# wanmeihuali/taichi_3d_gaussian_splatting

Hardware: NVIDIA H100
Metric: rendered Mpix/sec fwd+bwd @1080p, 1e6 Gaussians (higher is better)
Workload: dtype f32

## Files before the change

### taichi_3d_gaussian_splatting_b200/csrc/blend_bwd.cu

```cuda
#include "blend_bwd.cuh"

namespace gsb {

__device__ __forceinline__ void warp_transpose_reduce11(float (&v)[11], int lane) {
    {
        const bool hi = lane & 16;
#pragma unroll
        for (int i = 0; i < 5; ++i) {
            const float send = hi ? v[i] : v[i + 6];
            const float keep = hi ? v[i + 6] : v[i];
            v[i] = keep + __shfl_xor_sync(0xffffffffu, send, 16);
        }
        v[5] += __shfl_xor_sync(0xffffffffu, v[5], 16);
    }
    {
        const bool hi = lane & 8;
#pragma unroll
        for (int i = 0; i < 3; ++i) {
            const float send = hi ? v[i] : v[i + 3];
            const float keep = hi ? v[i + 3] : v[i];
            v[i] = keep + __shfl_xor_sync(0xffffffffu, send, 8);
        }
    }
    {
// ... 138 lines not shown
                            v[3] = vs0 * q1;
                            v[4] = vs1 * q1;
                            v[5] = aT * g0;
                            v[6] = aT * g1;
                            v[7] = aT * g2;
                            v[8] = a_grad * gp * (1.0f - opa) * opa;
                            v[9] = STATS ? sqrtf(vs0 * vs0 + vs1 * vs1) : 0.0f;
                        } else {
                            const float P = fast_alpha(d0, d1, (-0.5f * GSB_L2E) * r0.z, -GSB_L2E * r0.w,
                                                       (-0.5f * GSB_L2E) * r1.x, r1.y);
                            contributes = (idx < last) && (P >= 1.0f / 255.0f);
                            const float alpha = fminf(P, 0.99f);
                            const float inv = rcp_approx(1.0f - alpha);
                            const float Tn = T * inv;
                            const float aT = contributes ? alpha * Tn : 0.0f;
                            const float cg = fmaf(r2.z, g2, fmaf(r2.y, g1, r2.x * g0));
                            const float a_grad = contributes ? fmaf(cg, Tn, -(w0 * inv)) : 0.0f;
                            T = contributes ? Tn : T;
                            w0 = fmaf(cg, aT, w0);
                            const float G = a_grad * P;
                            const float vs0 = G * q0, vs1 = G * q1;
                            if (STATS) {
                                mag0 += fabsf(vs0);
                                mag1 += fabsf(vs1);
                            }
                            v[0] = vs0;
                            v[1] = vs1;
                            v[2] = vs0 * q0;
                            v[3] = vs0 * q1;
                            v[4] = vs1 * q1;
                            v[5] = aT * g0;
                            v[6] = aT * g1;
                            v[7] = aT * g2;
                            v[8] = G * r1.z;
                            v[9] = STATS ? sqrt_approx(vs0 * vs0 + vs1 * vs1) : 0.0f;
                        }
                        v[10] = (STATS && contributes) ? 1.0f : 0.0f;
                    }
                    if (lane == 0) GSB_EMU_COUNT(EC_BF_VISITS, 1);
                    GSB_EMU_COUNT(EC_BF_PAIRS, contributes ? 1 : 0);
                    if (__any_sync(0xffffffffu, contributes)) {
                        if (lane == 0) GSB_EMU_COUNT(EC_BF_VISITS_ANY, 1);
                        warp_transpose_reduce11(v, lane);
                        if (red_writer && (STATS || red_slot < 9))
                            atomicAdd(p.accum + (size_t)s_off[buf][j] * GSB_ACCUM_FLOATS + red_slot, v[0]);
                    }
                }
            }
        }
    }
    if (STATS) {
        p.mag_image[2 * pix] = mag0;
        p.mag_image[2 * pix + 1] = mag1;
    }
}

#ifndef GSB_HOST_EMU
static BlendBwdParams make_blend_bwd_params(const GsbBackwardArgs &a, const Workspace &ws);

int launch_blend_backward_work(const GsbBackwardArgs &a, const Workspace &ws, unsigned long long *counters_dev,
                               cudaStream_t stream) {
    BlendBwdParams p = make_blend_bwd_params(a, ws);
    p.work_counters = counters_dev;
    const int tiles = p.tiles_x * (a.camera_height / GSB_TILE_HEIGHT);
    if (tiles <= 0) return GSB_OK;
    return launch_blend_backward_count(p, tiles, stream);
}

static BlendBwdParams make_blend_bwd_params(const GsbBackwardArgs &a, const Workspace &ws) {
    BlendBwdParams p;
    p.H = a.camera_height;
    p.W = a.camera_width;
    p.tiles_x = a.camera_width / GSB_TILE_WIDTH;
    p.tile_start = ws.tile_start;
    p.tile_end = ws.tile_end;
    p.sorted_vals = ws.vals_b;
    p.records = ws.records;
    p.grad_image = a.grad_rasterized_image;
    p.acc_alpha = a.pixel_accumulated_alpha;
    p.last_effective = a.pixel_offset_of_last_effective_point;
    p.accum = a.accum;
    p.mag_image = a.magnitude_grad_viewspace_on_image;
    p.work_counters = nullptr;
    p.grad_depth = nullptr;
    p.depth = nullptr;
    p.grad_alpha = nullptr;
    return p;
}

int launch_blend_backward(const GsbBackwardArgs &a, const Workspace &ws, cudaStream_t stream, const float *grad_depth,
                          const float *depth, const float *grad_alpha, const GsbExtraFeatureArgs *ext) {
    BlendBwdParams p;
    p.H = a.camera_height;
    p.W = a.camera_width;
    p.tiles_x = a.camera_width / GSB_TILE_WIDTH;
    p.tile_start = ws.tile_start;
    p.tile_end = ws.tile_end;
    p.sorted_vals = ws.vals_b;
    p.records = ws.records;
    p.grad_image = a.grad_rasterized_image;
    p.acc_alpha = a.pixel_accumulated_alpha;
    p.last_effective = a.pixel_offset_of_last_effective_point;
    p.accum = a.accum;
    p.mag_image = a.magnitude_grad_viewspace_on_image;
    p.work_counters = nullptr;
    p.grad_depth = grad_depth;
    p.depth = depth;
    p.grad_alpha = grad_alpha;
    const BlendFeatureParams feat{ext ? ext->channels : 0, ws.point_id, ext ? ext->features : nullptr,
                                  ext ? ext->grad_rasterized : nullptr, ext ? ext->grad_features : nullptr};
    const int tiles = p.tiles_x * (a.camera_height / GSB_TILE_HEIGHT);
    if (tiles <= 0) return GSB_OK;
    if (a.flags & GSB_FLAG_BACKWARD_TRANSPOSED)
        return launch_blend_backward_transposed(p, tiles, (a.flags & GSB_FLAG_EXACT_EXP) != 0,
                                                (a.flags & GSB_FLAG_NO_HOOK_STATS) == 0, stream, grad_depth != nullptr,
                                                grad_alpha != nullptr, ext ? &feat : nullptr);
    const bool exact = (a.flags & GSB_FLAG_EXACT_EXP) != 0;
    if (a.flags & GSB_FLAG_NO_HOOK_STATS) {
        if (exact) blend_backward_kernel<true, false><<<tiles, GSB_TILE_PIXELS, 0, stream>>>(p);
        else blend_backward_kernel<false, false><<<tiles, GSB_TILE_PIXELS, 0, stream>>>(p);
    } else if (exact) {
        blend_backward_kernel<true><<<tiles, GSB_TILE_PIXELS, 0, stream>>>(p);
    } else {
        blend_backward_kernel<false><<<tiles, GSB_TILE_PIXELS, 0, stream>>>(p);
    }
    GSB_CUDA_CHECK(cudaGetLastError());
    return GSB_OK;
}
#endif

__device__ __forceinline__ void sh_basis(float dx, float dy, float dz, float (&sh)[16]) {
    const float dinv = 1.0f / sqrtf(dx * dx + dy * dy + dz * dz);
    dx *= dinv; dy *= dinv; dz *= dinv;
    sh[0] = 0.28209479177387814f;
    sh[1] = -0.48860251190291987f * dy;
    sh[2] = 0.48860251190291987f * dz;
    sh[3] = -0.48860251190291987f * dx;
    sh[4] = 1.0925484305920792f * dx * dy;
    sh[5] = -1.0925484305920792f * dy * dz;
    sh[6] = 0.94617469575755997f * dz * dz - 0.31539156525251999f;
    sh[7] = -1.0925484305920792f * dx * dz;
    sh[8] = 0.54627421529603959f * dx * dx - 0.54627421529603959f * dy * dy;
    sh[9] = 0.59004358992664352f * dy * (-3.0f * dx * dx + dy * dy);
    sh[10] = 2.8906114426405538f * dx * dy * dz;
    sh[11] = 0.45704579946446572f * dy * (1.0f - 5.0f * dz * dz);
    sh[12] = 0.3731763325901154f * dz * (5.0f * dz * dz - 3.0f);
    sh[13] = 0.45704579946446572f * dx * (1.0f - 5.0f * dz * dz);
    sh[14] = 1.4453057213202769f * dz * (dx * dx - dy * dy);
    sh[15] = 0.59004358992664352f * dx * (-dx * dx + 3.0f * dy * dy);
}

struct PointsBwdParams {
    long long N;
    const int *point_offset;
    const float4 *records;
    const float *point_in_camera;
    const float *accum;
    const PoseBlock *poses;
    const float *xyz;
    const float *features;
    const int *obj_id;
    const float *t_pc_cam;
    const float *K;
    int first_cleared;
    float q_f, s_f, a_f, c_f, h_f;
    float *grad_xyz;
    float *grad_feat;
    int *ctl_num_in_camera;
    int *ctl_num_pixels;
    float *ctl_vs_grad;
    float *ctl_vs_grad_avg;
    float *ctl_pos_grad;
    float *ctl_pos_grad_norm;
    const long long *skip_flag;
    float *grad_sum_compact;
    float *grad_color_compact;
};

#ifndef GSB_POINTS_THREADS
#define GSB_POINTS_THREADS 128
#endif
constexpr int PT_ROW = 60;
constexpr int PT_ROW_COMPACT = 20;
constexpr int POSE_VALUES = 12;
constexpr int INTR_VALUES = 6;
__device__ __forceinline__ void weighted_u_sigma(const float *U, const float *R, const float *es, float g00, float g01,
                                                 float g11, float *B0, float *B1) {
    float UM[6];
// ... 970 lines not shown
```

### taichi_3d_gaussian_splatting_b200/csrc/blend_bwd.cuh

```cuda
#pragma once
#include "common.cuh"

namespace gsb {

struct BlendBwdParams {
    int H, W, tiles_x;
    const int *tile_start;
    const int *tile_end;
    const int *sorted_vals;
    const float4 *records;
    const float *grad_image;
    const float *acc_alpha;
    const int *last_effective;
    float *accum;
    float *mag_image;
    unsigned long long *work_counters;
    const float *grad_depth;
    const float *depth;
    const float *grad_alpha;
};
struct BlendFeatureParams {
    int channels;
    const int *point_id;
    const float *features;
    const float *grad_feature_map;
    float *grad_features;
};
struct BlendBwdFeatParams : BlendBwdParams {
    BlendFeatureParams feat;
};
__device__ __forceinline__ BlendFeatureParams feature_params(const BlendBwdParams &) {
    return BlendFeatureParams{0, nullptr, nullptr, nullptr, nullptr};
}
__device__ __forceinline__ BlendFeatureParams feature_params(const BlendBwdFeatParams &p) { return p.feat; }

#ifdef GSB_HOST_EMU
__device__ __forceinline__ float ex2_approx_b(float x) { return exp2f(x); }
__device__ __forceinline__ float rcp_approx(float x) { return 1.0f / x; }
__device__ __forceinline__ float sqrt_approx(float x) { return sqrtf(x); }
#else
__device__ __forceinline__ float ex2_approx_b(float x) {
    float y;
    asm("ex2.approx.ftz.f32 %0, %1;" : "=f"(y) : "f"(x));
    return y;
}
__device__ __forceinline__ float rcp_approx(float x) {
    float y;
    asm("rcp.approx.ftz.f32 %0, %1;" : "=f"(y) : "f"(x));
    return y;
}
__device__ __forceinline__ float sqrt_approx(float x) {
    float y;
    asm("sqrt.approx.ftz.f32 %0, %1;" : "=f"(y) : "f"(x));
    return y;
}
#endif

int launch_blend_backward_transposed(const BlendBwdParams &p, int tiles, bool exact_exp, bool stats,
                                     cudaStream_t stream, bool depth = false, bool alpha = false,
                                     const BlendFeatureParams *feat = nullptr);
int launch_blend_backward_count(const BlendBwdParams &p, int tiles, cudaStream_t stream);

}
```

### taichi_3d_gaussian_splatting_b200/csrc/blend_bwd_transposed.cu

```cuda
#include <type_traits>

#include "blend_bwd.cuh"

namespace gsb {

#ifndef GSB_TB_CHUNK
#define GSB_TB_CHUNK 16
#endif
#ifndef GSB_TB_MIN_BLOCKS
#if GSB_TB_CHUNK == 8
#define GSB_TB_MIN_BLOCKS 4
#else
#define GSB_TB_MIN_BLOCKS 3
#endif
#endif
constexpr int TB_CHUNK = GSB_TB_CHUNK;
static_assert(TB_CHUNK == 8 || TB_CHUNK == 16, "a phase-2 lane takes whole rows of the 8 x 4 patch");
constexpr int TB_ROWS = TB_CHUNK / 8;
constexpr int TB_ROW = TB_CHUNK + 1;

struct TbWarp {
    float4 g[32];
    float4 chunk[3][TB_CHUNK];
    float2 x[32 * TB_ROW];
    int chunk_off[TB_CHUNK];
    unsigned char list[GSB_TILE_PIXELS];
};
struct TbShared {
    float4 rec[2 * 3 * GSB_TILE_PIXELS];
    TbWarp w[8];
    unsigned int bits[2][8][8];
    float2 origin;
    int max_last;
};
static_assert(2 * 32 * TB_ROW >= TB_CHUNK * GSB_ACCUM_FLOATS && GSB_ACCUM_FLOATS == 12,
              "the finished rows (3 float4 each) must fit into the exchange buffer");
static_assert(GSB_TB_MIN_BLOCKS * (sizeof(TbShared) + 1024) <= 228 * 1024,
              "the shared-memory image does not allow GSB_TB_MIN_BLOCKS CTAs per SM");

template <int CF>
struct TbFeat {
    int row[2][GSB_TILE_PIXELS];
    struct Warp {
        float4 g[32][CF / 4];
        float4 f[TB_CHUNK][CF / 4];
        int row[TB_CHUNK];
    } w[8];
};
constexpr int TB_FEAT_MIN_BLOCKS = 2;
constexpr int tb_min_blocks(int cf) { return cf == 0 ? GSB_TB_MIN_BLOCKS : TB_FEAT_MIN_BLOCKS; }
template <int CF>
constexpr size_t tb_smem_bytes() { return sizeof(TbShared) + (CF > 0 ? sizeof(TbFeat<(CF > 0 ? CF : 4)>) : 0); }
static_assert(sizeof(TbShared) % 16 == 0, "TbFeat starts 16-byte aligned");
static_assert(TB_FEAT_MIN_BLOCKS * (tb_smem_bytes<16>() + 1024) <= 228 * 1024,
              "the feature instantiations' shared-memory image does not allow TB_FEAT_MIN_BLOCKS CTAs per SM");

#ifdef GSB_HOST_EMU
static inline unsigned char *tb_dynamic_smem() { return simt_emu::dynamic_smem(); }
#else
extern __shared__ __align__(16) unsigned char gsb_tb_dynamic_smem[];
__device__ __forceinline__ unsigned char *tb_dynamic_smem() { return gsb_tb_dynamic_smem; }
#endif

#ifndef GSB_TB_P1_UNROLL
#define GSB_TB_P1_UNROLL 4
#endif
constexpr int TB_P1_UNROLL = GSB_TB_P1_UNROLL;
static_assert(TB_CHUNK % TB_P1_UNROLL == 0, "a full chunk is a whole number of phase-1 groups");
__device__ __forceinline__ void red_add_f32x4(float *addr, const float4 v) {
#ifdef GSB_HOST_EMU
    atomicAdd(addr, v.x);
    atomicAdd(addr + 1, v.y);
    atomicAdd(addr + 2, v.z);
    atomicAdd(addr + 3, v.w);
#else
    atomicAdd(reinterpret_cast<float4 *>(addr), v);
#endif
}
__device__ __forceinline__ float keep_if_contributing(float P, int idx, int last) {
#ifdef GSB_HOST_EMU
    return ((idx < last) && (P >= 1.0f / 255.0f)) ? P : 0.0f;
#else
    float r;
    asm("{\n"
        ".reg .pred p, q;\n"
        "setp.lt.s32 q, %2, %3;\n"
        "setp.ge.and.f32 p, %1, 0f3B808081, q;\n"
        "selp.f32 %0, %1, 0f00000000, p;\n"
        "}\n"
        : "=f"(r)
        : "f"(P), "r"(idx), "r"(last));
    return r;
#endif
}

template <int CF>
using TbParams = typename std::conditional<CF == 0, BlendBwdParams, BlendBwdFeatParams>::type;

template <bool EXACT_EXP, bool STATS, bool COUNT = false, bool DEPTH = false, bool ALPHA = false, int CF = 0>
__global__ void __launch_bounds__(GSB_TILE_PIXELS, tb_min_blocks(CF))
blend_backward_transposed_kernel(const TbParams<CF> p) {
    static_assert(!(COUNT && (DEPTH || ALPHA || CF)), "the work-counter diagnostic runs the default arithmetic only");
    static_assert(CF % 4 == 0 && CF <= 16, "features: whole float4 groups");
    TbShared &S = *reinterpret_cast<TbShared *>(tb_dynamic_smem());
    constexpr int NV = STATS ? 11 : 9;
    constexpr int CFW = CF > 0 ? CF : 4;
    constexpr int P1U = CF >= 16 ? 2 : TB_P1_UNROLL;
    TbFeat<CFW> &SF = *reinterpret_cast<TbFeat<CFW> *>(tb_dynamic_smem() + sizeof(TbShared));

    const int tile = blockIdx.x;
    const int tu = tile % p.tiles_x, tv = tile / p.tiles_x;
    const int tid = threadIdx.x, lane = tid & 31, warp = tid >> 5;
    const int pu = tu * GSB_TILE_WIDTH + (warp & 1) * 8 + (lane & 7);
    const int pv = tv * GSB_TILE_HEIGHT + (warp >> 1) * 4 + (lane >> 3);
    const float px = (float)pu + 0.5f, py = (float)pv + 0.5f;
    const size_t pix = (size_t)pv * p.W + pu;
    const int start = p.tile_start[tile];

    const int last = p.last_effective[pix];
    float T = 1.0f - p.acc_alpha[pix];
    float w0 = 0.0f, w1 = 0.0f, w2 = 0.0f;
    const float g0 = p.grad_image[3 * pix], g1 = p.grad_image[3 * pix + 1], g2 = p.grad_image[3 * pix + 2];
    float mag0 = 0.0f, mag1 = 0.0f;
    unsigned int n_visits = 0, n_pairs = 0;
    float gd = 0.0f, hd = 0.0f, w3 = 0.0f;
    if (DEPTH) {
        const float Sa = p.acc_alpha[pix];
        gd = Sa > 0.0f ? p.grad_depth[pix] / Sa : 0.0f;
        hd = EXACT_EXP ? p.depth[pix] : gd * p.depth[pix];
    }
    float ga = 0.0f;
    if (ALPHA) {
        const float gs = p.grad_alpha[pix];
        ga = EXACT_EXP ? gs * T : DEPTH ? gs - hd : gs;
    }
    TbWarp &Wp = S.w[warp];
    Wp.g[lane] = make_float4(g0, g1, g2, gd);
    float gf[CFW];
    float wF;
    typename TbFeat<CFW>::Warp &WF = SF.w[warp];
    const BlendFeatureParams fp = feature_params(p);
    const int C = CF > 0 ? fp.channels : 0;
    if constexpr (CF > 0) {
        wF = 0.0f;
        const float *src = fp.grad_feature_map + pix * C;
#pragma unroll
        for (int c = 0; c < CF; ++c) gf[c] = c < C ? src[c] : 0.0f;
#pragma unroll
        for (int c = 0; c < CF; c += 4) WF.g[lane][c / 4] = make_float4(gf[c], gf[c + 1], gf[c + 2], gf[c + 3]);
    }

    const int ci = lane % TB_CHUNK, row0 = (lane / TB_CHUNK) * TB_ROWS;
    float2 *const x = Wp.x;
    float4 *const fin = reinterpret_cast<float4 *>(x);
    unsigned char *const list = Wp.list;

    int warp_last = last;
#pragma unroll
    for (int d = 16; d > 0; d >>= 1) warp_last = max(warp_last, __shfl_xor_sync(0xffffffffu, warp_last, d));
    if (tid == 0) {
        S.max_last = start;
        S.origin = make_float2((float)(tu * GSB_TILE_WIDTH), (float)(tv * GSB_TILE_HEIGHT));
    }
    __syncthreads();
    if (lane == 0) atomicMax(&S.max_last, warp_last);
    __syncthreads();
    const int end = min(p.tile_end[tile], S.max_last);

    float4 *const ck0 = Wp.chunk[0], *const ck1 = Wp.chunk[1], *const ck2 = Wp.chunk[2];
    int *const ck_off = Wp.chunk_off;
    int have = 0;

    int buf = 0;
    for (int block_end = end;; block_end -= GSB_TILE_PIXELS, buf ^= 1) {
        const bool real = block_end > start;
        int count = 0;
        float4 *const s_r0 = S.rec + buf * 3 * GSB_TILE_PIXELS;
        float4 *const s_r1 = s_r0 + GSB_TILE_PIXELS, *const s_r2 = s_r0 + 2 * GSB_TILE_PIXELS;
        if (real) {
            const int block_start = max(block_end - GSB_TILE_PIXELS, start);
            {
                const int idx = block_end - 1 - tid;
                unsigned int mask = 0;
                if (idx >= block_start) {
                    const int o = __ldg(&p.sorted_vals[idx]);
                    const float4 *rec = p.records + 3 * (size_t)o;
                    const float4 r0 = __ldg(rec), r1 = __ldg(rec + 1);
                    if (EXACT_EXP) {
                        s_r0[tid] = r0;
                        s_r1[tid] = r1;
                    } else {
                        float4 f0, f1;
                        fast_planes(r0, r1, f0, f1);
                        s_r0[tid] = f0;
                        s_r1[tid] = f1;
                    }
                    float4 r2 = __ldg(rec + 2);
                    r2.w = __int_as_float(o);
                    s_r2[tid] = r2;
                    if constexpr (CF > 0) SF.row[buf][tid] = __ldg(&fp.point_id[o]);
                    mask = splat_patch_mask(r0.x, r0.y, r0.z, r0.w, r1.x, r1.y * r1.z, S.origin.x, S.origin.y);
                }
#pragma unroll
                for (int w = 0; w < 8; ++w) {
                    const unsigned int bits = __ballot_sync(0xffffffffu, (mask >> w) & 1u);
                    if (lane == 0) S.bits[buf][w][warp] = bits;
                }
            }
            __syncthreads();
            if (tid == 0) GSB_EMU_COUNT(EC_BATCHES, 1);
            if (block_start < warp_last) {
                const int skip = block_end - warp_last;
#pragma unroll
                for (int k = 0; k < 8; ++k) {
                    unsigned int bits = S.bits[buf][warp][k];
                    const int lo = skip - 32 * k;
                    if (lo >= 32) bits = 0u;
                    else if (lo > 0) bits &= ~((1u << lo) - 1u);
                    if ((bits >> lane) & 1u)
                        list[count + __popc(bits & ((1u << lane) - 1u))] = (unsigned char)(k * 32 + lane);
                    count += __popc(bits);
                }
                __syncwarp();
            }
        }

        int pos = 0;
#pragma unroll 1
        do {
            if (pos < count) {
                const int take = min(TB_CHUNK - have, count - pos);
                if (lane < take) {
                    const int j = list[pos + lane], slot = have + lane;
                    ck0[slot] = s_r0[j];
                    ck1[slot] = s_r1[j];
                    float4 r2 = s_r2[j];
                    ck_off[slot] = __float_as_int(r2.w);
                    r2.w = __int_as_float(block_end - 1 - j);
                    ck2[slot] = r2;
                    if constexpr (CF > 0) {
                        const int row = SF.row[buf][j];
                        WF.row[slot] = row;
                        const float *src = fp.features + (size_t)row * C;
#pragma unroll
                        for (int c = 0; c < CF; c += 4)
                            WF.f[slot][c / 4] = make_float4(c < C ? __ldg(src + c) : 0.0f, c + 1 < C ? __ldg(src + c + 1) : 0.0f,
                                                            c + 2 < C ? __ldg(src + c + 2) : 0.0f,
                                                            c + 3 < C ? __ldg(src + c + 3) : 0.0f);
                    }
                }
                have += take;
                pos += take;
                __syncwarp();
            }
            if (have == TB_CHUNK || (!real && have > 0)) {
                const int n = have;
                have = 0;
                if (COUNT) n_visits += (lane == 0) ? (unsigned int)n : 0u;
                if (lane == 0) {
                    GSB_EMU_COUNT(EC_TB_SPLATS, n);
                    GSB_EMU_COUNT(EC_TB_CHUNKS, 1);
                }
                const auto p1 = [&](const int i) -> float2 {
                    const float4 r0 = ck0[i];
                    const float4 r1 = ck1[i];
                    const float4 r2 = ck2[i];
                    const int idx = __float_as_int(r2.w);
                    const float d0 = px - r0.x, d1 = py - r0.y;
                    float sf = 0.0f;
                    if constexpr (CF > 0) {
#pragma unroll
                        for (int c = 0; c < CF; c += 4) {
                            const float4 f = WF.f[i][c / 4];
                            sf = fmaf(gf[c], f.x, sf);
                            sf = fmaf(gf[c + 1], f.y, sf);
                            sf = fmaf(gf[c + 2], f.z, sf);
                            sf = fmaf(gf[c + 3], f.w, sf);
                        }
                    }
                    float G, aT;
                    if (EXACT_EXP) {
                        const float q0 = r0.z * d0 + r0.w * d1;
                        const float q1 = r0.w * d0 + r1.x * d1;
                        const float gp = expf(-0.5f * (d0 * q0 + d1 * q1)) * r1.y;
                        const float prod_alpha = gp * r1.z;
                        const bool contributes = (idx < last) && (prod_alpha >= 1.0f / 255.0f);
                        const float alpha = fminf(prod_alpha, 0.99f);
                        const float inv = 1.0f / (1.0f - alpha);
                        const float Tn = T * inv;
                        aT = contributes ? alpha * Tn : 0.0f;
                        float a_grad = contributes ? (r2.x * Tn - w0 * inv) * g0 + (r2.y * Tn - w1 * inv) * g1 +
                                                         (r2.z * Tn - w2 * inv) * g2
                                                   : 0.0f;
                        if (DEPTH) {
                            const float e = r1.w - hd;
                            a_grad += contributes ? (e * Tn - w3 * inv) * gd : 0.0f;
                            w3 = fmaf(e, aT, w3);
                        }
                        if (ALPHA) a_grad += contributes ? ga * inv : 0.0f;
                        if constexpr (CF > 0) {
                            a_grad += contributes ? sf * Tn - wF * inv : 0.0f;
                            wF = fmaf(sf, aT, wF);
                        }
                        T = contributes ? Tn : T;
                        w0 = fmaf(r2.x, aT, w0);
                        w1 = fmaf(r2.y, aT, w1);
                        w2 = fmaf(r2.z, aT, w2);
                        G = a_grad * r1.z * gp;
                        if (STATS) {
                            mag0 += fabsf(G * q0);
                            mag1 += fabsf(G * q1);
                        }
                    } else {
                        float P = fast_alpha(d0, d1, r0.z, r0.w, r1.x, r1.y);
                        P = keep_if_contributing(P, idx, last);
                        const float alpha = fminf(P, 0.99f);
                        const float inv = rcp_approx(1.0f - alpha);
                        T *= inv;
                        aT = alpha * T;
                        float cg = fmaf(r2.z, g2, fmaf(r2.y, g1, ALPHA ? fmaf(r2.x, g0, ga) : r2.x * g0));
                        if (DEPTH) cg = ALPHA ? fmaf(gd, r1.w, cg) : fmaf(gd, r1.w, cg) - hd;
// ... 236 lines not shown
```

### taichi_3d_gaussian_splatting_b200/csrc/blend_fwd.cu

```cuda
#include <type_traits>

#include "common.cuh"

namespace gsb {

struct BlendFwdParams {
    int H, W, tiles_x;
    const int *tile_start;
    const int *tile_end;
    const int *sorted_vals;
    const float4 *records;
    float *image;
    float *depth;
    float *acc_alpha;
    int *last_effective;
    int *valid_count;
    unsigned long long *work_counters;
};
struct BlendFwdFeatParams : BlendFwdParams {
    int channels;
    const int *point_id;
    const float *features;
    float *out_features;
};
template <int CF>
using FwParams = typename std::conditional<CF == 0, BlendFwdParams, BlendFwdFeatParams>::type;
struct FwFeatureArgs {
    int channels;
    const int *point_id;
    const float *features;
    float *out_features;
};
__device__ __forceinline__ FwFeatureArgs feature_args(const BlendFwdParams &) { return FwFeatureArgs{0, nullptr, nullptr, nullptr}; }
__device__ __forceinline__ FwFeatureArgs feature_args(const BlendFwdFeatParams &p) {
    return FwFeatureArgs{p.channels, p.point_id, p.features, p.out_features};
}

#ifdef GSB_HOST_EMU
static inline float *fw_feature_smem() { return reinterpret_cast<float *>(simt_emu::dynamic_smem()); }
#else
extern __shared__ __align__(16) float gsb_fw_dynamic_smem[];
__device__ __forceinline__ float *fw_feature_smem() { return gsb_fw_dynamic_smem; }
#endif

__device__ __forceinline__ float ex2_approx(float x) { return ex2_mufu(x); }

__device__ __forceinline__ void count_if_blended(float wgt, int idx, int &cnt, int &last) {
#ifdef GSB_HOST_EMU
    if (wgt > 0.0f) {
        cnt += 1;
        last = idx;
    }
#else
    asm("{\n"
        ".reg .pred p;\n"
        "setp.gt.f32 p, %2, 0f00000000;\n"
        "@p add.s32 %0, %0, 1;\n"
        "@p mov.b32 %1, %3;\n"
        "}\n"
        : "+r"(cnt), "+r"(last)
        : "f"(wgt), "r"(idx));
#endif
}

#ifndef GSB_FWD_MIN_BLOCKS
#define GSB_FWD_MIN_BLOCKS 4
#endif
#ifndef GSB_FWD_UNROLL
#define GSB_FWD_UNROLL 8
#endif
constexpr int FW_UNROLL = GSB_FWD_UNROLL;
constexpr int FW_CHUNK = 32;
template <int CF>
__device__ __forceinline__ const float4 *fw_feature_row(int buf, int j) {
    return reinterpret_cast<const float4 *>(fw_feature_smem() + (buf * GSB_TILE_PIXELS + j) * CF);
}
constexpr int fw_min_blocks(int cf, bool exact_exp) { return cf == 0 ? GSB_FWD_MIN_BLOCKS : (cf <= 8 && !exact_exp) ? 3 : 2; }
constexpr int fw_feature_smem_bytes(int cf) { return 2 * GSB_TILE_PIXELS * cf * (int)sizeof(float); }

template <bool RGB_ONLY, bool EXACT_EXP, bool COUNT = false, int CF = 0>
__global__ void __launch_bounds__(GSB_TILE_PIXELS, fw_min_blocks(CF, EXACT_EXP))
blend_forward_kernel(const FwParams<CF> p) {
    static_assert(CF == 0 || (CF % 4 == 0 && !RGB_ONLY && !COUNT), "features: whole float4 groups, full outputs only");
    __shared__ float4 s_rec[2 * 3 * GSB_TILE_PIXELS];
    __shared__ unsigned int s_bits[2][8][8];
    __shared__ float4 s_chunk[8][3][FW_CHUNK];
    __shared__ unsigned char s_list[8][GSB_TILE_PIXELS];

    const int tile = blockIdx.x;
    const int tu = tile % p.tiles_x, tv = tile / p.tiles_x;
    const int tid = threadIdx.x, lane = tid & 31, warp = tid >> 5;
    const int pu = tu * GSB_TILE_WIDTH + (warp & 1) * 8 + (lane & 7);
    const int pv = tv * GSB_TILE_HEIGHT + (warp >> 1) * 4 + (lane >> 3);
    const float px = (float)pu + 0.5f, py = (float)pv + 0.5f;
    const float tile_x0 = (float)(tu * GSB_TILE_WIDTH), tile_y0 = (float)(tv * GSB_TILE_HEIGHT);
    const int start = p.tile_start[tile], end = p.tile_end[tile];

    float T = 1.0f, Tlive = 1.0f, C0 = 0.0f, C1 = 0.0f, C2 = 0.0f, D = 0.0f, Wt = 0.0f;
    int last = start, cnt = 0;
    unsigned int n_visits = 0, n_pairs = 0;
    unsigned int n_p84 = 0, n_p88 = 0, n_p164 = 0, n_p44 = 0;
    float4 *const ck0 = s_chunk[warp][0], *const ck1 = s_chunk[warp][1], *const ck2 = s_chunk[warp][2];
    unsigned char *const list = s_list[warp];
    const unsigned int lt_mask = (1u << lane) - 1u;
    constexpr int CFW = CF > 0 ? CF : 4;
    const FwFeatureArgs fa = feature_args(p);
    float F[CFW];
#pragma unroll
    for (int c = 0; c < CFW; ++c) F[c] = 0.0f;

    int buf = 0;
    for (int base = start; base < end; base += GSB_TILE_PIXELS, buf ^= 1) {
        float4 *const s_r0 = s_rec + buf * 3 * GSB_TILE_PIXELS;
        float4 *const s_r1 = s_r0 + GSB_TILE_PIXELS, *const s_r2 = s_r0 + 2 * GSB_TILE_PIXELS;
        const int idx = base + tid;
        unsigned int mask = 0;
        if (idx < end) {
            const int o = __ldg(&p.sorted_vals[idx]);
            const float4 *rec = p.records + 3 * (size_t)o;
            const float4 r0 = __ldg(rec), r1 = __ldg(rec + 1);
            if (EXACT_EXP) {
                s_r0[tid] = r0;
                s_r1[tid] = r1;
            } else {
                float4 f0, f1;
                fast_planes(r0, r1, f0, f1);
                s_r0[tid] = f0;
                s_r1[tid] = f1;
            }
            s_r2[tid] = __ldg(rec + 2);
            if constexpr (CF > 0) {
                const int C = fa.channels;
                const float *src = fa.features + (size_t)__ldg(&fa.point_id[o]) * C;
                float4 *dst = reinterpret_cast<float4 *>(fw_feature_smem() + (buf * GSB_TILE_PIXELS + tid) * CF);
#pragma unroll
                for (int c = 0; c < CF; c += 4)
                    dst[c / 4] = make_float4(c < C ? __ldg(src + c) : 0.0f, c + 1 < C ? __ldg(src + c + 1) : 0.0f,
                                             c + 2 < C ? __ldg(src + c + 2) : 0.0f, c + 3 < C ? __ldg(src + c + 3) : 0.0f);
            }
            mask = splat_patch_mask(r0.x, r0.y, r0.z, r0.w, r1.x, r1.y * r1.z, tile_x0, tile_y0);
            if (COUNT) {
                n_p84 += __popc(mask);
                n_p88 += __popc((mask | (mask >> 2)) & 0x33u);
                n_p164 += __popc((mask | (mask >> 1)) & 0x55u);
                const SplatReach rr = make_splat_reach(r0.z, r0.w, r1.x, r1.y * r1.z);
                if (rr.mode == 2) n_p44 += 16;
                else if (rr.mode == 1)
                    for (int q = 0; q < 16; ++q) {
                        const float X0 = tile_x0 + 4.0f * (q & 3) + 0.5f - r0.x, Y0 = tile_y0 + 4.0f * (q >> 2) + 0.5f - r0.y;
                        n_p44 += rect_reachable(rr, X0, X0 + 3.0f, Y0, Y0 + 3.0f) ? 1 : 0;
                    }
            }
        }
#pragma unroll
        for (int w = 0; w < 8; ++w) {
            const unsigned int bits = __ballot_sync(0xffffffffu, (mask >> w) & 1u);
            if (lane == 0) s_bits[buf][w][warp] = bits;
        }
        if (__syncthreads_and(!(T > 0.0f))) break;
        if (__all_sync(0xffffffffu, !(T > 0.0f))) continue;
        int count = 0;
#pragma unroll
        for (int k = 0; k < 8; ++k) {
            const unsigned int bits = s_bits[buf][warp][k];
            if ((bits >> lane) & 1u) list[count + __popc(bits & lt_mask)] = (unsigned char)(k * 32 + lane);
            count += __popc(bits);
        }
        __syncwarp();
#pragma unroll 1
        for (int pos = 0; pos < count; pos += FW_CHUNK) {
            const int n = min(FW_CHUNK, count - pos);
            if (lane < n) {
                const int j = list[pos + lane];
                ck0[lane] = s_r0[j];
                ck1[lane] = s_r1[j];
                float4 r2 = s_r2[j];
                r2.w = __int_as_float(base + j + 1);
                ck2[lane] = r2;
            }
            __syncwarp();
            if (COUNT) n_visits += (lane == 0) ? (unsigned int)n : 0u;
            if (lane == 0) GSB_EMU_COUNT(EC_FW_VISITS, n);
#pragma unroll FW_UNROLL
            for (int i = 0; i < n; ++i) {
                const float4 r0 = ck0[i];
                const float4 r1 = ck1[i];
                const float4 r2 = ck2[i];
                const float dx = px - r0.x, dy = py - r0.y;
                if (EXACT_EXP) {
                    const float power = -0.5f * (dx * dx * r0.z + dy * dy * r1.x) - dx * dy * r0.w;
                    float alpha = expf(power) * r1.y * r1.z;
                    if (!(alpha < 1.0f / 255.0f)) {
                        if (COUNT) n_pairs += T > 0.0f ? 1u : 0u;
                        GSB_EMU_COUNT(EC_FW_PAIRS, 1);
                        alpha = fminf(alpha, 0.99f);
                        const float nT = T * (1.0f - alpha);
                        if (nT >= 0.0001f) {
                            last = __float_as_int(r2.w);
                            C0 += r2.x * alpha * T;
                            C1 += r2.y * alpha * T;
                            C2 += r2.z * alpha * T;
                            if (!RGB_ONLY) {
                                D += r1.w * alpha * T;
                                Wt += alpha * T;
                                cnt += 1;
                            }
                            if constexpr (CF > 0) {
                                const float4 *fi = fw_feature_row<CF>(buf, __float_as_int(r2.w) - 1 - base);
#pragma unroll
                                for (int c = 0; c < CF; c += 4) {
                                    const float4 f = fi[c / 4];
                                    F[c] += f.x * alpha * T;
                                    F[c + 1] += f.y * alpha * T;
                                    F[c + 2] += f.z * alpha * T;
                                    F[c + 3] += f.w * alpha * T;
                                }
                            }
                            T = nT;
                            Tlive = nT;
                        } else {
                            T = 0.0f;
                        }
                    }
                } else {
                    float P = fast_alpha(dx, dy, r0.z, r0.w, r1.x, r1.y);
                    P = (P < 1.0f / 255.0f) ? 0.0f : P;
                    const float alpha = fminf(P, 0.99f);
                    const float nT = T * (1.0f - alpha);
                    const bool ok = nT >= 0.0001f;
                    const float wgt = ok ? alpha * T : 0.0f;
                    if (COUNT) n_pairs += (P != 0.0f && T > 0.0f) ? 1u : 0u;
                    GSB_EMU_COUNT(EC_FW_PAIRS, (P != 0.0f && T > 0.0f) ? 1 : 0);
                    C0 = fmaf(r2.x, wgt, C0);
                    C1 = fmaf(r2.y, wgt, C1);
                    C2 = fmaf(r2.z, wgt, C2);
                    if (!RGB_ONLY) {
                        D = fmaf(r1.w, wgt, D);
                        Wt += wgt;
                        count_if_blended(wgt, __float_as_int(r2.w), cnt, last);
                    }
                    if constexpr (CF > 0) {
                        const float4 *fi = fw_feature_row<CF>(buf, __float_as_int(r2.w) - 1 - base);
#pragma unroll
                        for (int c = 0; c < CF; c += 4) {
                            const float4 f = fi[c / 4];
                            F[c] = fmaf(f.x, wgt, F[c]);
                            F[c + 1] = fmaf(f.y, wgt, F[c + 1]);
                            F[c + 2] = fmaf(f.z, wgt, F[c + 2]);
                            F[c + 3] = fmaf(f.w, wgt, F[c + 3]);
                        }
                    }
                    T = ok ? nT : -fabsf(T);
                }
            }
            __syncwarp();
            if (__all_sync(0xffffffffu, !(T > 0.0f))) break;
        }
    }
    const size_t pix = (size_t)pv * p.W + pu;
    p.image[3 * pix] = C0;
    p.image[3 * pix + 1] = C1;
    p.image[3 * pix + 2] = C2;
    if (!RGB_ONLY) {
        p.depth[pix] = D / fmaxf(Wt, 1e-6f);
        p.acc_alpha[pix] = 1.0f - (EXACT_EXP ? Tlive : fabsf(T));
        p.last_effective[pix] = last;
        p.valid_count[pix] = cnt;
    }
    if constexpr (CF > 0) {
        const int C = fa.channels;
#pragma unroll
        for (int c = 0; c < CF; ++c)
            if (c < C) fa.out_features[pix * C + c] = F[c];
    }
    if (COUNT) {
#pragma unroll
        for (int d = 16; d > 0; d >>= 1) {
            n_visits += __shfl_xor_sync(0xffffffffu, n_visits, d);
            n_pairs += __shfl_xor_sync(0xffffffffu, n_pairs, d);
            n_p84 += __shfl_xor_sync(0xffffffffu, n_p84, d);
            n_p88 += __shfl_xor_sync(0xffffffffu, n_p88, d);
            n_p164 += __shfl_xor_sync(0xffffffffu, n_p164, d);
            n_p44 += __shfl_xor_sync(0xffffffffu, n_p44, d);
        }
        if (lane == 0) {
            atomicAdd(p.work_counters, (unsigned long long)n_visits);
            atomicAdd(p.work_counters + 1, (unsigned long long)n_pairs);
            atomicAdd(p.work_counters + 2, (unsigned long long)n_p84);
            atomicAdd(p.work_counters + 3, (unsigned long long)n_p88);
            atomicAdd(p.work_counters + 4, (unsigned long long)n_p164);
            atomicAdd(p.work_counters + 5, (unsigned long long)n_p44);
        }
    }
}

#ifndef GSB_HOST_EMU
template <bool EXACT_EXP, int CF>
static int launch_fwd_features(const BlendFwdFeatParams &p, int tiles, cudaStream_t stream) {
    static bool configured = false;
    if (!configured) {
        GSB_CUDA_CHECK(cudaFuncSetAttribute(blend_forward_kernel<false, EXACT_EXP, false, CF>,
                                            cudaFuncAttributeMaxDynamicSharedMemorySize, fw_feature_smem_bytes(CF)));
        configured = true;
    }
    blend_forward_kernel<false, EXACT_EXP, false, CF><<<tiles, GSB_TILE_PIXELS, fw_feature_smem_bytes(CF), stream>>>(p);
    GSB_CUDA_CHECK(cudaGetLastError());
    return GSB_OK;
}

template <int CF>
static int launch_fwd_features(const BlendFwdFeatParams &p, int tiles, bool exact, cudaStream_t stream) {
    return exact ? launch_fwd_features<true, CF>(p, tiles, stream) : launch_fwd_features<false, CF>(p, tiles, stream);
}

int launch_blend_forward(const GsbForwardArgs &a, const Workspace &ws, cudaStream_t stream, const GsbExtraFeatureArgs *ext) {
    BlendFwdParams p;
    p.H = a.camera_height;
    p.W = a.camera_width;
    p.tiles_x = a.camera_width / GSB_TILE_WIDTH;
    p.tile_start = ws.tile_start;
    p.tile_end = ws.tile_end;
    p.sorted_vals = ws.vals_b;
    p.records = ws.records;
    p.image = a.rasterized_image;
    p.depth = a.rasterized_depth;
    p.acc_alpha = a.pixel_accumulated_alpha;
    p.last_effective = a.pixel_offset_of_last_effective_point;
    p.valid_count = a.pixel_valid_point_count;
    p.work_counters = nullptr;
    const int tiles = p.tiles_x * (a.camera_height / GSB_TILE_HEIGHT);
    if (tiles <= 0) return GSB_OK;
    const bool exact = (a.flags & GSB_FLAG_EXACT_EXP) != 0;
    if (ext) {
        BlendFwdFeatParams fp;
        static_cast<BlendFwdParams &>(fp) = p;
        fp.channels = ext->channels;
        fp.point_id = ws.point_id;
        fp.features = ext->features;
        fp.out_features = ext->rasterized;
        const int C = ext->channels;
        return C <= 4 ? launch_fwd_features<4>(fp, tiles, exact, stream)
             : C <= 8 ? launch_fwd_features<8>(fp, tiles, exact, stream)
                      : launch_fwd_features<16>(fp, tiles, exact, stream);
    }
    if (a.rgb_only) {
        if (exact) blend_forward_kernel<true, true><<<tiles, GSB_TILE_PIXELS, 0, stream>>>(p);
        else blend_forward_kernel<true, false><<<tiles, GSB_TILE_PIXELS, 0, stream>>>(p);
    } else {
        if (exact) blend_forward_kernel<false, true><<<tiles, GSB_TILE_PIXELS, 0, stream>>>(p);
        else blend_forward_kernel<false, false><<<tiles, GSB_TILE_PIXELS, 0, stream>>>(p);
    }
    GSB_CUDA_CHECK(cudaGetLastError());
    return GSB_OK;
}

int launch_blend_forward_count(const GsbForwardArgs &a, const Workspace &ws, unsigned long long *counters_dev,
                               cudaStream_t stream) {
    BlendFwdParams p;
    p.H = a.camera_height;
    p.W = a.camera_width;
    p.tiles_x = a.camera_width / GSB_TILE_WIDTH;
    p.tile_start = ws.tile_start;
    p.tile_end = ws.tile_end;
    p.sorted_vals = ws.vals_b;
    p.records = ws.records;
    p.image = a.rasterized_image;
    p.depth = a.rasterized_depth;
    p.acc_alpha = a.pixel_accumulated_alpha;
    p.last_effective = a.pixel_offset_of_last_effective_point;
    p.valid_count = a.pixel_valid_point_count;
    p.work_counters = counters_dev;
    const int tiles = p.tiles_x * (a.camera_height / GSB_TILE_HEIGHT);
    if (tiles <= 0) return GSB_OK;
    blend_forward_kernel<false, false, true><<<tiles, GSB_TILE_PIXELS, 0, stream>>>(p);
    GSB_CUDA_CHECK(cudaGetLastError());
    return GSB_OK;
}
#endif

}
```

### taichi_3d_gaussian_splatting_b200/csrc/common.cuh

```cuda
#pragma once
#include <cuda_runtime.h>
#include <stdint.h>

#include "../../include/gsb200.h"

#define GSB_TILE_PIXELS (GSB_TILE_WIDTH * GSB_TILE_HEIGHT)

namespace gsb {

void set_error(const char *fmt, ...);
#define GSB_CUDA_CHECK(expr)                                                                   \
    do {                                                                                       \
        cudaError_t _e = (expr);                                                               \
        if (_e != cudaSuccess) {                                                               \
            gsb::set_error("%s failed: %s (%s:%d)", #expr, cudaGetErrorString(_e), __FILE__,   \
                           __LINE__);                                                          \
            return GSB_ECUDA;                                                                  \
        }                                                                                      \
    } while (0)

enum Counter { CNT_M = 0, CNT_K = 1, CNT_OVERFLOW = 2, CNT_MAX_DEPTH_KEY = 4 };
enum Ticket { TICKET_SCAN = 0, TICKET_SORT0 = 1  };

struct PoseBlock {
// ... 103 lines not shown
constexpr int SCAN_BLOCK_THREADS = GSB_SCAN_THREADS;

#if defined(__CUDACC__) || defined(GSB_HOST_EMU)
#ifdef GSB_HOST_EMU
template <int BYTE_OFFSET>
inline float4 lds128(unsigned int saddr) {
    return *reinterpret_cast<const float4 *>(simt_emu::smem_anchor() + (long long)(int)saddr + BYTE_OFFSET);
}
inline unsigned int smem_u32(const void *p) {
    return (unsigned int)(int)(reinterpret_cast<const char *>(p) - simt_emu::smem_anchor());
}
inline float rcp_fast(float x) { return 1.0f / x; }
#else
template <int BYTE_OFFSET>
__device__ __forceinline__ float4 lds128(unsigned int saddr) {
    float4 v;
    asm volatile("ld.shared.v4.f32 {%0, %1, %2, %3}, [%4+%5];"
                 : "=f"(v.x), "=f"(v.y), "=f"(v.z), "=f"(v.w)
                 : "r"(saddr), "n"(BYTE_OFFSET));
    return v;
}
__device__ __forceinline__ unsigned int smem_u32(const void *p) {
    unsigned int a = (unsigned int)__cvta_generic_to_shared(p);
    asm volatile("" : "+r"(a));
    return a;
}
#endif

struct SplatReach {
    float a, b2, c;
    float nb_ic, nb_ia;
    float t2;
    int mode;
};
#ifndef GSB_HOST_EMU
__device__ __forceinline__ float rcp_fast(float x) {
    float y;
    asm("rcp.approx.ftz.f32 %0, %1;" : "=f"(y) : "f"(x));
    return y;
}
#endif
__device__ __forceinline__ float quad_form(const SplatReach &r, float dx, float dy) {
    return fmaf(dx, fmaf(r.b2, dy, r.a * dx), r.c * dy * dy);
}
__device__ __forceinline__ SplatReach make_splat_reach(float a, float b, float c, float rescale_times_opacity) {
    SplatReach r;
    r.a = a; r.b2 = 2.0f * b; r.c = c;
    const float ro = rescale_times_opacity;
    r.nb_ic = -b * rcp_fast(c);
    r.nb_ia = -b * rcp_fast(a);
    r.t2 = fmaf(2.0f * 1.002f, __logf(fmaxf(255.0f * ro, 1.0f)), 1e-3f);
    const float det = a * c - b * b;
    if (!(ro == ro) || !(det > 0.0f) || !(a > 0.0f) || !(c > 0.0f)) r.mode = 2;
    else if (ro < (1.0f / 255.0f) * 0.999f) r.mode = 0;
    else r.mode = 1;
    return r;
}
__device__ __forceinline__ bool rect_reachable(const SplatReach &r, float X0, float X1, float Y0, float Y1) {
    if (X0 <= 0.0f && X1 >= 0.0f && Y0 <= 0.0f && Y1 >= 0.0f) return true;
    const float ya = fminf(fmaxf(r.nb_ic * X0, Y0), Y1);
    const float yb = fminf(fmaxf(r.nb_ic * X1, Y0), Y1);
    const float xa = fminf(fmaxf(r.nb_ia * Y0, X0), X1);
    const float xb = fminf(fmaxf(r.nb_ia * Y1, X0), X1);
    const float best = fminf(fminf(quad_form(r, X0, ya), quad_form(r, X1, yb)),
                             fminf(quad_form(r, xa, Y0), quad_form(r, xb, Y1)));
    return !(best > r.t2);
}

__device__ __forceinline__ unsigned int splat_patch_mask(float u, float v, float a, float b, float c,
                                                         float rescale_times_opacity, float tile_x0,
                                                         float tile_y0) {
    const SplatReach r = make_splat_reach(a, b, c, rescale_times_opacity);
    if (r.mode == 0) return 0u;
    if (r.mode == 2) return 0xFFu;
    unsigned int m = 0;
#pragma unroll
    for (int w = 0; w < 8; ++w) {
        const float X0 = tile_x0 + 8.0f * (w & 1) + 0.5f - u;
        const float Y0 = tile_y0 + 4.0f * (w >> 1) + 0.5f - v;
        if (rect_reachable(r, X0, X0 + 7.0f, Y0, Y0 + 3.0f)) m |= 1u << w;
    }
    return m;
}
#endif

#if defined(__CUDACC__) || defined(GSB_HOST_EMU)
constexpr float GSB_L2E = 1.4426950408889634f;
#ifdef GSB_HOST_EMU
__device__ __forceinline__ float ex2_mufu(float x) { return exp2f(x); }
#else
__device__ __forceinline__ float ex2_mufu(float x) {
    float y;
    asm("ex2.approx.ftz.f32 %0, %1;" : "=f"(y) : "f"(x));
    return y;
}
#endif
__device__ __forceinline__ float fast_alpha(float dx, float dy, float A, float B, float C, float ro) {
    return ex2_mufu(fmaf(dx, fmaf(A, dx, B * dy), (C * dy) * dy)) * ro;
}
__device__ __forceinline__ void fast_planes(const float4 r0, const float4 r1, float4 &s0, float4 &s1) {
    s0 = make_float4(r0.x, r0.y, (-0.5f * GSB_L2E) * r0.z, -GSB_L2E * r0.w);
    s1 = make_float4((-0.5f * GSB_L2E) * r1.x, r1.y * r1.z, 1.0f - r1.z, r1.w);
}
#endif

struct LensParams {
    int model;
    float k[5];
    float r2_max;
};
#if defined(__CUDACC__) || defined(GSB_HOST_EMU)
template <int MODEL>
__device__ __forceinline__ void lens_distort(const float *k, float xn, float yn, float &ox, float &oy, float *D) {
    const float r2 = xn * xn + yn * yn;
    if (MODEL == GSB_LENS_OPENCV) {
        const float k1 = k[0], k2 = k[1], p1 = k[2], p2 = k[3], k3 = k[4];
        const float rad1 = r2 * (k1 + r2 * (k2 + r2 * k3));
        const float rad = 1.0f + rad1;
        const float drad = k1 + r2 * (2.0f * k2 + r2 * (3.0f * k3));
        ox = xn * rad1 + 2.0f * p1 * xn * yn + p2 * (r2 + 2.0f * xn * xn);
        oy = yn * rad1 + p1 * (r2 + 2.0f * yn * yn) + 2.0f * p2 * xn * yn;
        const float off = 2.0f * xn * yn * drad + 2.0f * (p1 * xn + p2 * yn);
        D[0] = rad + 2.0f * xn * xn * drad + 2.0f * p1 * yn + 6.0f * p2 * xn;
        D[1] = off;
        D[2] = off;
        D[3] = rad + 2.0f * yn * yn * drad + 6.0f * p1 * yn + 2.0f * p2 * xn;
    } else {
        float A, Ar;
        if (r2 < 0.04f) {
            A = 1.0f + r2 * (-1.0f / 3.0f + r2 * (1.0f / 5.0f + r2 * (-1.0f / 7.0f + r2 * (1.0f / 9.0f + r2 * (-1.0f / 11.0f)))));
            Ar = -2.0f / 3.0f + r2 * (4.0f / 5.0f + r2 * (-6.0f / 7.0f + r2 * (8.0f / 9.0f + r2 * (-10.0f / 11.0f))));
        } else {
            const float r = sqrtf(r2);
            A = atanf(r) / r;
            Ar = (1.0f / (1.0f + r2) - A) / r2;
        }
        const float t = A * A * r2;
        const float P = 1.0f + t * (k[0] + t * (k[1] + t * (k[2] + t * k[3])));
        const float dP = k[0] + t * (2.0f * k[1] + t * (3.0f * k[2] + t * (4.0f * k[3])));
        const float s = A * P;
        const float g = Ar * P + 2.0f * A * A * dP / (1.0f + r2);
        ox = (s - 1.0f) * xn;
        oy = (s - 1.0f) * yn;
        D[0] = s + g * xn * xn;
        D[1] = g * xn * yn;
        D[2] = D[1];
        D[3] = s + g * yn * yn;
    }
}
template <int MODEL>
__device__ __forceinline__ void lens_coefficient_grad(float xn, float yn, float gx, float gy, float w00, float w01, float w11,
                                                      float *out) {
    const float r2 = xn * xn + yn * yn;
    const float pos = gx * xn + gy * yn;
    const float tr = w00 + w11;
    const float quad = w00 * xn * xn + w01 * xn * yn + w11 * yn * yn;
    if (MODEL == GSB_LENS_OPENCV) {
        const float r4 = r2 * r2;
        out[0] = r2 * (pos + tr) + 2.0f * quad;
        out[1] = r4 * (pos + tr) + 4.0f * r2 * quad;
        out[2] = gx * (2.0f * xn * yn) + gy * (r2 + 2.0f * yn * yn) + 2.0f * w00 * yn + 2.0f * w01 * xn + 6.0f * w11 * yn;
        out[3] = gx * (r2 + 2.0f * xn * xn) + gy * (2.0f * xn * yn) + 6.0f * w00 * xn + 2.0f * w01 * yn + 2.0f * w11 * xn;
        out[4] = r4 * r2 * (pos + tr) + 6.0f * r4 * quad;
    } else {
        float A, Ar;
        if (r2 < 0.04f) {
// ... 224 lines not shown
```

Before: 1299.

## Record per-tile contributor lists in forward pass and replay them in backward

The forward blend kernel now records, per tile, which sorted splats actually contributed to some warp's 8x4 patch. It stores them as a compacted list of (index, warp mask) keys plus record offsets in spare workspace buffers (keys_c/vals_c), with a sentinel giving the count. The transposed backward kernel walks this compacted list instead of the raw sorted range. This drops the per-splat patch-mask computation and the max-last-effective reduction, and skips splats that never contributed. The cost is extra bookkeeping in the forward pass (contribution bitmasks, warp OR reduction, shared atomics, global writes). It also relies on the workspace buffers not being clobbered between forward and backward.

```diff
diff --git a/taichi_3d_gaussian_splatting_b200/csrc/blend_bwd.cu b/taichi_3d_gaussian_splatting_b200/csrc/blend_bwd.cu
--- a/taichi_3d_gaussian_splatting_b200/csrc/blend_bwd.cu
+++ b/taichi_3d_gaussian_splatting_b200/csrc/blend_bwd.cu
@@ -244,6 +244,8 @@
     p.accum = a.accum;
     p.mag_image = a.magnitude_grad_viewspace_on_image;
     p.work_counters = nullptr;
+    p.list_key = static_cast<const unsigned int *>(ws.keys_c);
+    p.list_off = ws.vals_c;
     p.grad_depth = nullptr;
     p.depth = nullptr;
     p.grad_alpha = nullptr;
@@ -266,6 +268,8 @@
     p.accum = a.accum;
     p.mag_image = a.magnitude_grad_viewspace_on_image;
     p.work_counters = nullptr;
+    p.list_key = static_cast<const unsigned int *>(ws.keys_c);
+    p.list_off = ws.vals_c;
     p.grad_depth = grad_depth;
     p.depth = depth;
     p.grad_alpha = grad_alpha;
diff --git a/taichi_3d_gaussian_splatting_b200/csrc/blend_bwd.cuh b/taichi_3d_gaussian_splatting_b200/csrc/blend_bwd.cuh
--- a/taichi_3d_gaussian_splatting_b200/csrc/blend_bwd.cuh
+++ b/taichi_3d_gaussian_splatting_b200/csrc/blend_bwd.cuh
@@ -18,6 +18,8 @@
     const float *grad_depth;
     const float *depth;
     const float *grad_alpha;
+    const unsigned int *list_key = nullptr;
+    const int *list_off = nullptr;
 };
 struct BlendFeatureParams {
     int channels;
diff --git a/taichi_3d_gaussian_splatting_b200/csrc/blend_bwd_transposed.cu b/taichi_3d_gaussian_splatting_b200/csrc/blend_bwd_transposed.cu
--- a/taichi_3d_gaussian_splatting_b200/csrc/blend_bwd_transposed.cu
+++ b/taichi_3d_gaussian_splatting_b200/csrc/blend_bwd_transposed.cu
@@ -29,9 +29,9 @@
 struct TbShared {
     float4 rec[2 * 3 * GSB_TILE_PIXELS];
     TbWarp w[8];
+    int idx[2][GSB_TILE_PIXELS];
     unsigned int bits[2][8][8];
     float2 origin;
-    int max_last;
 };
 static_assert(2 * 32 * TB_ROW >= TB_CHUNK * GSB_ACCUM_FLOATS && GSB_ACCUM_FLOATS == 12,
               "the finished rows (3 float4 each) must fit into the exchange buffer");
@@ -155,35 +155,39 @@
     float4 *const fin = reinterpret_cast<float4 *>(x);
     unsigned char *const list = Wp.list;
 
-    int warp_last = last;
-#pragma unroll
-    for (int d = 16; d > 0; d >>= 1) warp_last = max(warp_last, __shfl_xor_sync(0xffffffffu, warp_last, d));
-    if (tid == 0) {
-        S.max_last = start;
-        S.origin = make_float2((float)(tu * GSB_TILE_WIDTH), (float)(tv * GSB_TILE_HEIGHT));
-    }
-    __syncthreads();
-    if (lane == 0) atomicMax(&S.max_last, warp_last);
-    __syncthreads();
-    const int end = min(p.tile_end[tile], S.max_last);
+    if (tid == 0) S.origin = make_float2((float)(tu * GSB_TILE_WIDTH), (float)(tv * GSB_TILE_HEIGHT));
+    const int len = p.tile_end[tile] - start;
+    const bool raw = p.list_key == nullptr || len > GSB_CLIST_MAX_TILE;
+    int n_entries = len;
+    if (len > 0 && !raw && p.list_key[start + len - 1] == 0u) n_entries = p.list_off[start + len - 1];
 
     float4 *const ck0 = Wp.chunk[0], *const ck1 = Wp.chunk[1], *const ck2 = Wp.chunk[2];
     int *const ck_off = Wp.chunk_off;
     int have = 0;
 
     int buf = 0;
-    for (int block_end = end;; block_end -= GSB_TILE_PIXELS, buf ^= 1) {
-        const bool real = block_end > start;
+    for (int block_end = n_entries;; block_end -= GSB_TILE_PIXELS, buf ^= 1) {
+        const bool real = block_end > 0;
         int count = 0;
         float4 *const s_r0 = S.rec + buf * 3 * GSB_TILE_PIXELS;
         float4 *const s_r1 = s_r0 + GSB_TILE_PIXELS, *const s_r2 = s_r0 + 2 * GSB_TILE_PIXELS;
         if (real) {
-            const int block_start = max(block_end - GSB_TILE_PIXELS, start);
+            const int block_start = max(block_end - GSB_TILE_PIXELS, 0);
             {
-                const int idx = block_end - 1 - tid;
+                const int e = block_end - 1 - tid;
                 unsigned int mask = 0;
-                if (idx >= block_start) {
-                    const int o = __ldg(&p.sorted_vals[idx]);
+                if (e >= block_start) {
+                    int idx, o;
+                    if (raw) {
+                        idx = start + e;
+                        o = __ldg(&p.sorted_vals[idx]);
+                        mask = 0xFFu;
+                    } else {
+                        const unsigned int key = __ldg(&p.list_key[start + e]);
+                        o = __ldg(&p.list_off[start + e]);
+                        idx = start + (int)(key >> 8);
+                        mask = key & 0xFFu;
+                    }
                     const float4 *rec = p.records + 3 * (size_t)o;
                     const float4 r0 = __ldg(rec), r1 = __ldg(rec + 1);
                     if (EXACT_EXP) {
@@ -198,8 +202,8 @@
                     float4 r2 = __ldg(rec + 2);
                     r2.w = __int_as_float(o);
                     s_r2[tid] = r2;
+                    S.idx[buf][tid] = idx;
                     if constexpr (CF > 0) SF.row[buf][tid] = __ldg(&fp.point_id[o]);
-                    mask = splat_patch_mask(r0.x, r0.y, r0.z, r0.w, r1.x, r1.y * r1.z, S.origin.x, S.origin.y);
                 }
 #pragma unroll
                 for (int w = 0; w < 8; ++w) {
@@ -209,20 +213,13 @@
             }
             __syncthreads();
             if (tid == 0) GSB_EMU_COUNT(EC_BATCHES, 1);
-            if (block_start < warp_last) {
-                const int skip = block_end - warp_last;
-#pragma unroll
-                for (int k = 0; k < 8; ++k) {
-                    unsigned int bits = S.bits[buf][warp][k];
-                    const int lo = skip - 32 * k;
-                    if (lo >= 32) bits = 0u;
-                    else if (lo > 0) bits &= ~((1u << lo) - 1u);
-                    if ((bits >> lane) & 1u)
-                        list[count + __popc(bits & ((1u << lane) - 1u))] = (unsigned char)(k * 32 + lane);
-                    count += __popc(bits);
-                }
-                __syncwarp();
+#pragma unroll
+            for (int k = 0; k < 8; ++k) {
+                const unsigned int bits = S.bits[buf][warp][k];
+                if ((bits >> lane) & 1u) list[count + __popc(bits & ((1u << lane) - 1u))] = (unsigned char)(k * 32 + lane);
+                count += __popc(bits);
             }
+            __syncwarp();
         }
 
         int pos = 0;
@@ -236,7 +233,7 @@
                     ck1[slot] = s_r1[j];
                     float4 r2 = s_r2[j];
                     ck_off[slot] = __float_as_int(r2.w);
-                    r2.w = __int_as_float(block_end - 1 - j);
+                    r2.w = __int_as_float(S.idx[buf][j]);
                     ck2[slot] = r2;
                     if constexpr (CF > 0) {
                         const int row = SF.row[buf][j];
diff --git a/taichi_3d_gaussian_splatting_b200/csrc/blend_fwd.cu b/taichi_3d_gaussian_splatting_b200/csrc/blend_fwd.cu
--- a/taichi_3d_gaussian_splatting_b200/csrc/blend_fwd.cu
+++ b/taichi_3d_gaussian_splatting_b200/csrc/blend_fwd.cu
@@ -16,6 +16,8 @@
     int *last_effective;
     int *valid_count;
     unsigned long long *work_counters;
+    unsigned int *list_key = nullptr;
+    int *list_off = nullptr;
 };
 struct BlendFwdFeatParams : BlendFwdParams {
     int channels;
@@ -45,8 +47,9 @@
 
 __device__ __forceinline__ float ex2_approx(float x) { return ex2_mufu(x); }
 
-__device__ __forceinline__ void count_if_blended(float wgt, int idx, int &cnt, int &last) {
+__device__ __forceinline__ void count_if_blended(float wgt, int idx, int &cnt, int &last, unsigned int &vb) {
 #ifdef GSB_HOST_EMU
+    vb = 2u * vb + (wgt > 0.0f ? 1u : 0u);
     if (wgt > 0.0f) {
         cnt += 1;
         last = idx;
@@ -54,12 +57,24 @@
 #else
     asm("{\n"
         ".reg .pred p;\n"
-        "setp.gt.f32 p, %2, 0f00000000;\n"
+        "setp.gt.f32 p, %3, 0f00000000;\n"
+        "shl.b32 %2, %2, 1;\n"
         "@p add.s32 %0, %0, 1;\n"
-        "@p mov.b32 %1, %3;\n"
+        "@p mov.b32 %1, %4;\n"
+        "@p or.b32 %2, %2, 1;\n"
         "}\n"
-        : "+r"(cnt), "+r"(last)
+        : "+r"(cnt), "+r"(last), "+r"(vb)
         : "f"(wgt), "r"(idx));
+#endif
+}
+
+__device__ __forceinline__ unsigned int warp_or(unsigned int v) {
+#ifdef GSB_HOST_EMU
+    unsigned int r = 0u;
+    for (int b = 0; b < 32; ++b) r |= __ballot_sync(0xffffffffu, (v >> b) & 1u) != 0u ? 1u << b : 0u;
+    return r;
+#else
+    return __reduce_or_sync(0xffffffffu, v);
 #endif
 }
 
@@ -86,6 +101,8 @@
     __shared__ unsigned int s_bits[2][8][8];
     __shared__ float4 s_chunk[8][3][FW_CHUNK];
     __shared__ unsigned char s_list[8][GSB_TILE_PIXELS];
+    constexpr bool LIST = !RGB_ONLY;
+    __shared__ unsigned int s_contrib[LIST ? 3 : 1][GSB_TILE_PIXELS];
 
     const int tile = blockIdx.x;
     const int tu = tile % p.tiles_x, tv = tile / p.tiles_x;
@@ -108,6 +125,31 @@
     float F[CFW];
 #pragma unroll
     for (int c = 0; c < CFW; ++c) F[c] = 0.0f;
+    const bool listing = LIST && p.list_key != nullptr && end - start <= GSB_CLIST_MAX_TILE;
+    int n_listed = 0;
+    bool emit_last = end > start;
+    if (LIST) s_contrib[0][tid] = 0u;
+    const auto emit = [&](const int pb, const int pbuf, const unsigned int *contrib) {
+        unsigned int mine = 0u, word = 0u;
+        int before = 0, total = 0;
+#pragma unroll
+        for (int g = 0; g < 8; ++g) {
+            const unsigned int c = contrib[32 * g + lane];
+            const unsigned int b = __ballot_sync(0xffffffffu, c != 0u);
+            if (g == warp) {
+                mine = c;
+                word = b;
+            }
+            before += g < warp ? __popc(b) : 0;
+            total += __popc(b);
+        }
+        if (mine != 0u) {
+            const int k = start + n_listed + before + __popc(word & lt_mask);
+            p.list_key[k] = ((unsigned int)(pb + tid - start) << 8) | mine;
+            p.list_off[k] = __float_as_int(s_rec[(pbuf * 3 + 2) * GSB_TILE_PIXELS + tid].w);
+        }
+        n_listed += total;
+    };
 
     int buf = 0;
     for (int base = start; base < end; base += GSB_TILE_PIXELS, buf ^= 1) {
@@ -128,7 +170,9 @@
                 s_r0[tid] = f0;
                 s_r1[tid] = f1;
             }
-            s_r2[tid] = __ldg(rec + 2);
+            float4 r2 = __ldg(rec + 2);
+            if (LIST) r2.w = __int_as_float(o);
+            s_r2[tid] = r2;
             if constexpr (CF > 0) {
                 const int C = fa.channels;
                 const float *src = fa.features + (size_t)__ldg(&fa.point_id[o]) * C;
@@ -157,7 +201,16 @@
             const unsigned int bits = __ballot_sync(0xffffffffu, (mask >> w) & 1u);
             if (lane == 0) s_bits[buf][w][warp] = bits;
         }
-        if (__syncthreads_and(!(T > 0.0f))) break;
+        const bool all_saturated = __syncthreads_and(!(T > 0.0f));
+        const int kb = (base - start) / GSB_TILE_PIXELS;
+        if (listing) {
+            if (kb > 0) emit(base - GSB_TILE_PIXELS, buf ^ 1, s_contrib[(kb + 2) % 3]);
+            s_contrib[(kb + 1) % 3][tid] = 0u;
+        }
+        if (all_saturated) {
+            emit_last = false;
+            break;
+        }
         if (__all_sync(0xffffffffu, !(T > 0.0f))) continue;
         int count = 0;
 #pragma unroll
@@ -181,6 +234,7 @@
             __syncwarp();
             if (COUNT) n_visits += (lane == 0) ? (unsigned int)n : 0u;
             if (lane == 0) GSB_EMU_COUNT(EC_FW_VISITS, n);
+            unsigned int vb = 0u;
 #pragma unroll FW_UNROLL
             for (int i = 0; i < n; ++i) {
                 const float4 r0 = ck0[i];
@@ -188,6 +242,7 @@
                 const float4 r2 = ck2[i];
                 const float dx = px - r0.x, dy = py - r0.y;
                 if (EXACT_EXP) {
+                    if (LIST) vb = 2u * vb + (T > 0.0f ? 1u : 0u);
                     const float power = -0.5f * (dx * dx * r0.z + dy * dy * r1.x) - dx * dy * r0.w;
                     float alpha = expf(power) * r1.y * r1.z;
                     if (!(alpha < 1.0f / 255.0f)) {
@@ -237,7 +292,7 @@
                     if (!RGB_ONLY) {
                         D = fmaf(r1.w, wgt, D);
                         Wt += wgt;
-                        count_if_blended(wgt, __float_as_int(r2.w), cnt, last);
+                        count_if_blended(wgt, __float_as_int(r2.w), cnt, last, vb);
                     }
                     if constexpr (CF > 0) {
                         const float4 *fi = fw_feature_row<CF>(buf, __float_as_int(r2.w) - 1 - base);
@@ -253,8 +308,24 @@
                     T = ok ? nT : -fabsf(T);
                 }
             }
+            if (LIST) {
+                vb = warp_or(vb);
+                const int kb = (base - start) / GSB_TILE_PIXELS;
+                if (lane < n && ((vb >> (n - 1 - lane)) & 1u)) atomicOr(&s_contrib[kb % 3][list[pos + lane]], 1u << warp);
+            }
             __syncwarp();
             if (__all_sync(0xffffffffu, !(T > 0.0f))) break;
+        }
+    }
+    if (listing) {
+        if (emit_last) {
+            const int kb = (end - 1 - start) / GSB_TILE_PIXELS;
+            __syncthreads();
+            emit(start + kb * GSB_TILE_PIXELS, kb & 1, s_contrib[kb % 3]);
+        }
+        if (tid == 0 && n_listed < end - start) {
+            p.list_key[end - 1] = 0u;
+            p.list_off[end - 1] = n_listed;
         }
     }
     const size_t pix = (size_t)pv * p.W + pu;
@@ -328,6 +399,8 @@
     p.last_effective = a.pixel_offset_of_last_effective_point;
     p.valid_count = a.pixel_valid_point_count;
     p.work_counters = nullptr;
+    p.list_key = static_cast<unsigned int *>(ws.keys_c);
+    p.list_off = ws.vals_c;
     const int tiles = p.tiles_x * (a.camera_height / GSB_TILE_HEIGHT);
     if (tiles <= 0) return GSB_OK;
     const bool exact = (a.flags & GSB_FLAG_EXACT_EXP) != 0;
@@ -370,6 +443,8 @@
     p.last_effective = a.pixel_offset_of_last_effective_point;
     p.valid_count = a.pixel_valid_point_count;
     p.work_counters = counters_dev;
+    p.list_key = static_cast<unsigned int *>(ws.keys_c);
+    p.list_off = ws.vals_c;
     const int tiles = p.tiles_x * (a.camera_height / GSB_TILE_HEIGHT);
     if (tiles <= 0) return GSB_OK;
     blend_forward_kernel<false, false, true><<<tiles, GSB_TILE_PIXELS, 0, stream>>>(p);
diff --git a/taichi_3d_gaussian_splatting_b200/csrc/common.cuh b/taichi_3d_gaussian_splatting_b200/csrc/common.cuh
--- a/taichi_3d_gaussian_splatting_b200/csrc/common.cuh
+++ b/taichi_3d_gaussian_splatting_b200/csrc/common.cuh
@@ -209,6 +209,8 @@
     }
     return m;
 }
+
+constexpr int GSB_CLIST_MAX_TILE = 1 << 24;
 #endif
 
 #if defined(__CUDACC__) || defined(GSB_HOST_EMU)
```

New measurement: 1329, median of 6. 1.02x the previous value.
